# jankammeth/BA-path-planning

Hardware: AMD Instinct MI355X
Metric: SCP iterations/sec (N agents x K waypoints) (higher is better)
Workload: dtype f64

## Files before the change

### ba-path-planning_amd/csrc/scp_common.h

```cpp
#pragma once
#include <hip/hip_runtime.h>

#include <cstdarg>
#include <cstdint>
#include <cstdio>
#include <cstring>

#include "scp_hip.h"

struct scp_stats_mirror {
  scp_pair_stats stats;
  unsigned long long n_spec;
  double pts[6];
  double rel[64];
  volatile unsigned long long seq;
};

constexpr int SCP_SMALL_MAX_WG = 2048;

struct scp_ctx {
  int device;
  int n_cu;
  hipStream_t stream;
  char err[512];
// ... 1 lines not shown
  double* h_scratch;
  double* h_scratch_dev;
  hipEvent_t ev0, ev1;
  hipEvent_t pair_ev0, pair_ev1;
  bool pair_timed;
  bool pair_ran;
  bool last_pass_small;
  double* tm_scratch;
  size_t tm_bytes;
  uint32_t* cmp_map;
  size_t cmp_map_bytes;
  uint32_t* cmp_tot;
  size_t cmp_tot_bytes;
  scp_stats_mirror* h_mirror;
  scp_stats_mirror* d_mirror;
  unsigned long long mirror_seq;
  unsigned long long* wg_part;
  uint32_t* wg_rows;
  size_t wg_rows_bytes;
  unsigned* d_ticket;
  int timing;
  int small_pass;
  unsigned long long rel_seq;
  void* gen_ws;
  size_t gen_ws_bytes;
  void* sep_ws;
  size_t sep_ws_bytes;
  unsigned long long* solved;
  bool solved_ran[2];
  int* h_gen_flag;
  int* d_gen_flag;
  void* asg_ws;
  size_t asg_ws_bytes;
};

static inline int scp_fail(scp_ctx* ctx, int code, const char* fmt, ...) {
  if (ctx) {
    va_list ap;
    va_start(ap, fmt);
    vsnprintf(ctx->err, sizeof(ctx->err), fmt, ap);
    va_end(ap);
  }
  return code;
}

#define SCP_HIP_CHECK(ctx, call)                                                                     \
  do {                                                                                               \
    hipError_t e_ = (call);                                                                          \
    if (e_ != hipSuccess)                                                                            \
      return scp_fail((ctx), SCP_ERR_HIP, "%s failed: %s (%s:%d)", #call, hipGetErrorString(e_),    \
                      __FILE__, __LINE__);                                                           \
  } while (0)

#define SCP_REQUIRE(ctx, cond, ...)                                   \
  do {                                                                \
    if (!(cond)) return scp_fail((ctx), SCP_ERR_INVALID, __VA_ARGS__); \
  } while (0)

static inline int64_t scp_pairs(int N) { return (int64_t)N * (N - 1) / 2; }
static inline int scp_cdiv(int64_t a, int64_t b) { return (int)((a + b - 1) / b); }

int scp_ctx_ensure_bytes(scp_ctx* ctx, void** buf, size_t* have, size_t need);

hipError_t scp_raise_lds_limit(int device, const void* kernel, size_t bytes);

bool scp_wait_host_word(volatile unsigned long long* word, unsigned long long seq, int timeout_s);

int scp_check_pair_range(scp_ctx* ctx, int N, int K, int D, int64_t q_begin, int64_t q_end);

int scp_ctx_wait_stats(scp_ctx* ctx, scp_pair_stats* out);

int scp_violations_from_solution(scp_ctx* ctx, int N, int K, int D, double R, double h, int64_t q_begin, int64_t q_end,
                                 const double* pos_prev, const double* x_tm, const double* p0, const double* v0, double* x_out,
                                 double* pos_out, double feas_tol, int64_t* new_rows, int64_t new_cap, uint32_t* sel_bitmap,
                                 scp_pair_stats* stats, const double* rel_prev ,
                                 int64_t* spec_rows , int64_t spec_cap,
                                 uint32_t* spec_bitmap, double spec_margin, bool* fused);
void scp_ctx_mirror_rel(scp_ctx* ctx, int64_t n, double* out);
int scp_select_from_solution(scp_ctx* ctx, int N, int K, int D, double R, double h, int64_t q_begin, int64_t q_end,
                             const double* x_tm, const double* p0, const double* v0, double* x_out, double* pos_out,
                             double margin, int64_t* sel_rows, int64_t sel_cap, uint32_t* sel_bitmap, scp_pair_stats* stats,
                             bool* fused);
int scp_launch_kinematics_copy(scp_ctx* ctx, int N, int K, int D, double h, const double* acc, const double* p0,
                               const double* v0, double* pos_out, double* vel_out, double* acc_copy);
const double* scp_qp_solution_tm(const scp_qp* qp);

int scp_qp_reset_add_rows_at(scp_qp* qp, const double* x0, int64_t n, const int64_t* rows, const double* pos_prev,
                             const double* p0, const double* v0, double R);
int scp_qp_add_rows_from_pass(scp_qp* qp, int64_t n, const int64_t* rows, const double* eta, const double* l_col,
                              int64_t q_begin, int64_t q_end);

int scp_launch_add_rows_at(scp_ctx* ctx, int N, int K, int D, int64_t base, int64_t n, const int64_t* rows,
                           const double* pos_prev, const double* p0, const double* v0, double R, double h, const double* Qx,
                           int64_t* w_row, int* wk, int* wi, int* wj, double* weta, double* wl, double* zc, double* yc);

int scp_launch_gemm(scp_ctx* ctx, int use_mfma, int R, int M, int C, double alpha, const double* A,
                    const double* X, double beta, double* Y);
int scp_launch_to_time_major(scp_ctx* ctx, int N, int K, int D, const double* src, double* dst);
int scp_launch_from_time_major(scp_ctx* ctx, int N, int K, int D, const double* src, double* dst);
// ... 5 lines not shown
```

### ba-path-planning_amd/csrc/scp_ctx.hip

```cpp
#include "scp_common.h"
#include "scp_traj_device.h"

#include <sys/prctl.h>
#include <time.h>

#include <atomic>
#include <chrono>
#include <cmath>
#include <cstdlib>
#include <map>
#include <mutex>
#include <utility>

extern "C" int scp_abi_version(void) { return SCP_ABI_VERSION; }

extern "C" int scp_ctx_create(int device, void* hip_stream, scp_ctx** out) {
  if (!out) return SCP_ERR_INVALID;
  *out = nullptr;
  if (hipSetDevice(device) != hipSuccess) return SCP_ERR_HIP;
  scp_ctx* ctx = new scp_ctx();
  memset(ctx, 0, sizeof(*ctx));
  ctx->device = device;
  ctx->stream = (hipStream_t)hip_stream;
  ctx->timing = 1;
  ctx->small_pass = getenv("SCP_NO_SMALL_PASS") ? 0 : 1;
  if (hipDeviceGetAttribute(&ctx->n_cu, hipDeviceAttributeMultiprocessorCount, device) != hipSuccess) ctx->n_cu = 0;
  if (hipMalloc(&ctx->d_scratch, 72 * sizeof(double)) != hipSuccess ||
      hipMemset(ctx->d_scratch, 0, 72 * sizeof(double)) != hipSuccess ||
      hipHostMalloc(&ctx->h_scratch, 72 * sizeof(double)) != hipSuccess ||
      memset(ctx->h_scratch, 0, 72 * sizeof(double)) == nullptr ||
      hipHostGetDevicePointer((void**)&ctx->h_scratch_dev, ctx->h_scratch, 0) != hipSuccess ||
      hipHostMalloc(&ctx->h_mirror, sizeof(scp_stats_mirror)) != hipSuccess ||
      hipHostGetDevicePointer((void**)&ctx->d_mirror, ctx->h_mirror, 0) != hipSuccess ||
      hipEventCreate(&ctx->ev0) != hipSuccess || hipEventCreate(&ctx->ev1) != hipSuccess ||
      hipEventCreate(&ctx->pair_ev0) != hipSuccess || hipEventCreate(&ctx->pair_ev1) != hipSuccess ||
      hipMalloc(&ctx->wg_part, 4 * SCP_SMALL_MAX_WG * sizeof(unsigned long long)) != hipSuccess ||
      hipMalloc(&ctx->d_ticket, 64) != hipSuccess || hipMemset(ctx->d_ticket, 0, 64) != hipSuccess) {
    delete ctx;
    return SCP_ERR_HIP;
  }
  ctx->solved = (unsigned long long*)(ctx->d_ticket + 12);
  *out = ctx;
  return SCP_OK;
}

extern "C" int scp_ctx_set_option(scp_ctx* ctx, const char* key, int value) {
  if (!ctx || !key) return SCP_ERR_INVALID;
  if (strcmp(key, "kernel_timing") == 0) {
    ctx->timing = value ? 1 : 0;
    if (!ctx->timing) ctx->pair_timed = false;
    return SCP_OK;
  }
  if (strcmp(key, "single_launch_passes") == 0) {
    ctx->small_pass = value ? 1 : 0;
    return SCP_OK;
  }
  return scp_fail(ctx, SCP_ERR_INVALID, "ctx_set_option: unknown key '%s'", key);
}
// ... 116 lines not shown
```

### ba-path-planning_amd/csrc/scp_kernels.hip

```cpp
#include "scp_common.h"
#include "scp_compact_device.h"
#include "scp_pair_device.h"
#include "scp_traj_device.h"
#include "scp_wave_device.h"

#include <algorithm>
#include <cstdlib>

__device__ inline void pair_stats_init(scp_pair_stats* s) {
  s->min_dist = __longlong_as_double(0x7FF0000000000000LL);
  s->first_violation = 0xFFFFFFFFFFFFFFFFULL;
  s->n_selected = 0;
  s->max_violation = -__longlong_as_double(0x7FF0000000000000LL);
}

constexpr int PAIR_THREADS = 256;
constexpr int PAIR_STEPS = 16;
template <bool USE_LDS, int MODE>
struct PairUnroll {
  static constexpr int value = (USE_LDS && MODE != 2 ) ? 2 : 4;
};
constexpr int PAIR_ROWS = PAIR_THREADS * PAIR_STEPS * 2;
constexpr int PAIR_LDS_SLICE_BYTES = 16 * 1024;
constexpr int PAIR_LDS_Q_OFF = PAIR_LDS_SLICE_BYTES / 8;
// ... 808 lines not shown
        f = red_u[w] < f ? red_u[w] : f;
      }
      const double cur = __hip_atomic_load(&a.stats->min_dist, __ATOMIC_RELAXED, __HIP_MEMORY_SCOPE_AGENT);
      if (m < cur) atomic_min_pos_double(&a.stats->min_dist, m);
      if ((a.ablate & 1) && my_maxv == 12345.678) a.stats->max_violation = my_maxv;
      if (f != 0xFFFFFFFFFFFFFFFFULL) {
        const unsigned long long curf = __hip_atomic_load((unsigned long long*)&a.stats->first_violation,
                                                          __ATOMIC_RELAXED, __HIP_MEMORY_SCOPE_AGENT);
        if (f < curf) atomicMin((unsigned long long*)&a.stats->first_violation, f);
      }
    } else {
      double m = red_d[0];
#pragma unroll
      for (int w = 1; w < PAIR_THREADS / 64; ++w) m = fmax(m, red_d[w]);
      const double cur = __hip_atomic_load(&a.stats->max_violation, __ATOMIC_RELAXED, __HIP_MEMORY_SCOPE_AGENT);
      if (m > cur) atomic_max_double(&a.stats->max_violation, m);
    }
  }
#ifdef SCP_PHASE_PROFILE
  if (threadIdx.x == 0) {
    const unsigned wg = blockIdx.y * gridDim.x + blockIdx.x;
    if (wg < (unsigned)SCP_PAIR_CLK_WGS) {
      scp_pair_clk[2 * wg] = __builtin_amdgcn_s_memtime() - clk_c0;
      scp_pair_clk[2 * wg + 1] = __builtin_amdgcn_s_memrealtime() - clk_t0;
      scp_pair_t0[wg] = clk_t0;
    }
  }
#endif
}

__global__ __launch_bounds__(256) void pair_prep_delta_kernel(int N, int K, int D, const double* __restrict__ pos_prev,
                                                               const double* __restrict__ pos_new,
                                                               double* __restrict__ P_tm, double* __restrict__ dP_tm,
                                                               scp_pair_stats* __restrict__ stats) {
  const int64_t t = (int64_t)blockIdx.x * 256 + threadIdx.x;
  const int64_t C = (int64_t)N * D;
  if (t == 0) pair_stats_init(stats);
  if (t >= C * K) return;
  const int k = (int)(t / C);
  const int c = (int)(t % C);
  const int i = c / D, d = c % D;
  const int64_t g = ((int64_t)i * K + k) * D + d;
  const double pp = pos_prev[g];
  P_tm[t] = pp;
  dP_tm[t] = pos_new[g] - pp;
}

__global__ __launch_bounds__(CMP_THREADS) void compact_count_kernel(const uint32_t* __restrict__ map, int64_t words,
                                                                     uint32_t* __restrict__ block_tot) {
  const int64_t w0 = (int64_t)blockIdx.x * CMP_WORDS + (int64_t)threadIdx.x * CMP_WPT;
  int c = 0;
#pragma unroll
  for (int i = 0; i < CMP_WPT; ++i)
    if (w0 + i < words) c += __popc(map[w0 + i]);
  int tot;
  block_exclusive_scan(c, &tot);
  if (threadIdx.x == 0) block_tot[blockIdx.x] = (uint32_t)tot;
}

__global__ __launch_bounds__(CMP_THREADS) void compact_scan_kernel(uint32_t* __restrict__ block_tot, int nblocks,
                                                                    scp_pair_stats* __restrict__ stats,
                                                                    scp_stats_mirror* __restrict__ mirror,
                                                                    unsigned long long seq) {
  int carry = 0;
  for (int b0 = 0; b0 < nblocks; b0 += CMP_THREADS) {
    const int b = b0 + threadIdx.x;
    const int v = b < nblocks ? (int)block_tot[b] : 0;
    int tot;
    const int ex = block_exclusive_scan(v, &tot);
    if (b < nblocks) block_tot[b] = (uint32_t)(carry + ex);
    carry += tot;
  }
  if (threadIdx.x == 0) {
    stats->n_selected = (unsigned long long)carry;
    publish_stats(stats, (unsigned long long)carry, mirror, seq);
  }
}

// ... 176 lines not shown
  const int64_t slots = (int64_t)std::max(per_cu, 1) * ctx->n_cu;
  PairItems& it = a.items;
  it = PairItems{};
  const int64_t big_per_k = scp_cdiv(nq + 1, PAIR_ROWS);
  int nk_quarter = 0, nk_half = 0;
  if (big_per_k * K > slots) {
    nk_quarter = (int)((slots * (PAIR_ROWS / 4) + nq / 2) / nq);
    nk_half = (int)((slots * (PAIR_ROWS / 2) + nq / 2) / nq);
    if (nk_quarter + nk_half > K / 2) nk_quarter = nk_half = 0;
  }
#ifdef SCP_PHASE_PROFILE
  if (const char* e = getenv("SCP_PAIR_TAIL")) {
    int h_ = 0, q_ = 0;
    if (sscanf(e, "%d %d", &h_, &q_) == 2 && h_ >= 0 && q_ >= 0 && h_ + q_ < K) { nk_half = h_; nk_quarter = q_; }
  }
#endif
  const int nk[3] = {K - nk_half - nk_quarter, nk_half, nk_quarter};
  const int st[3] = {PAIR_STEPS, PAIR_STEPS / 2, PAIR_STEPS / 4};
  int k0 = 0, item0 = 0;
  for (int c = 0; c < 3; ++c) {
    if (nk[c] <= 0) continue;
    const int m = it.n_classes++;
    it.item0[m] = item0;
    it.k0[m] = k0;
    it.steps[m] = st[c];
    it.cpk[m] = (int)scp_cdiv(nq + 1, (int64_t)2 * PAIR_THREADS * st[c]);
    item0 += nk[c] * it.cpk[m];
    k0 += nk[c];
  }
  it.n_items = item0;
  return SCP_OK;
}

static int launch_large_pass(scp_ctx* ctx, int mode, PairArgs& a, const PassMarks& marks, const double* pos, const double* p0,
                             const double* v0) {
  const int N = a.N, K = a.K, D = a.D;
  const int64_t nq = a.q_end - a.q_begin;
  ctx->last_pass_small = false;
  const size_t slice = ((size_t)N * K * D + 1) & ~(size_t)1;
  const int rc = scp_ctx_ensure_bytes(ctx, (void**)&ctx->tm_scratch, &ctx->tm_bytes, 2 * slice * sizeof(double));
  if (rc) return rc;
  double* P_tm = mode != MODE_VIOLATIONS ? ctx->tm_scratch : nullptr;
  double* Q_tm = (mode != MODE_CHECK && mode != MODE_SELECT) ? ctx->tm_scratch + slice : nullptr;
  const dim3 prep_grid(scp_cdiv((int64_t)N * K * D, 256));
  const bool clear = marks.kind == PassMarks::REPLACE;
  if (mode == MODE_VIOL_RECOMPUTE)
    hipLaunchKernelGGL(pair_prep_delta_kernel, prep_grid, dim3(256), 0, ctx->stream, N, K, D, pos, p0, P_tm, Q_tm, a.stats);
  else
    hipLaunchKernelGGL(pair_prep_kernel, prep_grid, dim3(256), 0, ctx->stream, N, K, D, a.h, pos, p0, v0, P_tm, Q_tm,
                       a.stats, clear ? marks.bitmap : nullptr, clear ? a.words : (int64_t)0);
  a.P_tm = P_tm;
  a.Q_tm = Q_tm;
  if (nq <= 0) return SCP_OK;
  const size_t slice_bytes = (size_t)N * D * sizeof(double);
  const bool two_slices = mode == MODE_LINEARIZE || mode == MODE_VIOL_RECOMPUTE;
  const bool use_lds = slice_bytes <= (size_t)(two_slices ? 1 : 2) * PAIR_LDS_SLICE_BYTES && ((N * D) % 2 == 0) && !(a.ablate & 2);
  const size_t lds_bytes = !use_lds ? 0 : (two_slices ? PAIR_LDS_SLICE_BYTES + slice_bytes : slice_bytes);
  const PairKernel kern = pair_kernel(mode, D, use_lds, false);
  dim3 grid(scp_cdiv(nq + 1, PAIR_ROWS), K);
  if (mode == MODE_LINEARIZE) {
    const int rc_items = split_linearize_items(ctx, a, kern, lds_bytes);
    if (rc_items) return rc_items;
    grid = dim3((unsigned)a.items.n_items, 1);
  }
  return launch_pair_kernel(ctx, kern, grid, lds_bytes, a);
}

static int pair_pass(scp_ctx* ctx, int mode, PairArgs& a, const PassMarks& marks, const double* pos, const double* p0,
                     const double* v0) {
  if (marks.kind != PassMarks::NONE) {
    const int rc = ensure_cmp(ctx, a.words);
    if (rc) return rc;
  }
  a.bitmap = marks.bitmap;
  a.mark = marks.kind == PassMarks::MERGE ? ctx->cmp_map : marks.bitmap;
#ifdef SCP_PHASE_PROFILE
  const char* abl = getenv("SCP_PAIR_ABLATE");
  a.ablate = abl ? atoi(abl) : 0;
#endif
  if (pair_mode_has_small(mode) && small_pass_ok(ctx, a.N, a.K, a.D, a.q_end - a.q_begin, small_pass_slices(mode, a)))
    return launch_small_pass(ctx, mode, a, marks, pos, p0);
  const int rc = launch_large_pass(ctx, mode, a, marks, pos, p0, v0);
  if (rc || marks.kind == PassMarks::NONE) return rc;
  return launch_compaction(ctx, a.mark, a.words, a.q_end - a.q_begin, a.q_begin, a.pairs, marks.rows, marks.cap,
                           marks.kind == PassMarks::MERGE ? marks.bitmap : nullptr, a.stats);
}

#ifdef SCP_PHASE_PROFILE
extern "C" int scp_debug_small_clocks(unsigned long long* out, int n) {
  if (n > 16) n = 16;
  return hipMemcpyFromSymbol(out, HIP_SYMBOL(scp_small_clk), (size_t)n * sizeof(unsigned long long)) == hipSuccess ? 0 : 1;
}
extern "C" int scp_debug_pair_starts(unsigned long long* out, int n) {
  if (n > SCP_PAIR_CLK_WGS) n = SCP_PAIR_CLK_WGS;
  return hipMemcpyFromSymbol(out, HIP_SYMBOL(scp_pair_t0), (size_t)n * sizeof(unsigned long long)) == hipSuccess ? 0 : 1;
}
extern "C" int scp_debug_pair_clocks(unsigned long long* out, int n) {
  if (n > 2 * SCP_PAIR_CLK_WGS) n = 2 * SCP_PAIR_CLK_WGS;
  return hipMemcpyFromSymbol(out, HIP_SYMBOL(scp_pair_clk), (size_t)n * sizeof(unsigned long long)) == hipSuccess ? 0 : 1;
}
#endif

extern "C" int scp_ctx_last_pair_ms(scp_ctx* ctx, float* ms) {
  if (!ctx || !ms) return SCP_ERR_INVALID;
  if (!ctx->pair_timed && ctx->pair_ran) {
    *ms = 0.f;
    return SCP_OK;
  }
  if (!ctx->pair_timed) return scp_fail(ctx, SCP_ERR_STATE, "no pairwise pass has run yet");
  SCP_HIP_CHECK(ctx, hipEventSynchronize(ctx->pair_ev1));
  SCP_HIP_CHECK(ctx, hipEventElapsedTime(ms, ctx->pair_ev0, ctx->pair_ev1));
  return SCP_OK;
}

// ... 55 lines not shown
  if (!ctx) return SCP_ERR_INVALID;
  const int rc = scp_check_pair_range(ctx, N, K, D, q_begin, q_end);
  if (rc) return rc;
  SCP_REQUIRE(ctx, eta && l_col && pos && p0 && v0 && sel_bitmap && stats && (new_rows || new_cap == 0),
              "collision_violations: null pointer");
  PairArgs a = pair_args(N, K, D, 0.0, h, q_begin, q_end, stats);
  a.eta = const_cast<double*>(eta); a.l = const_cast<double*>(l_col); a.margin = feas_tol;
  return pair_pass(ctx, MODE_VIOLATIONS, a, {PassMarks::MERGE, new_rows, new_cap, sel_bitmap}, pos, p0, v0);
}

extern "C" int scp_collision_violations_at(scp_ctx* ctx, int N, int K, int D, double R, int64_t q_begin, int64_t q_end,
                                           const double* pos_prev, const double* pos_new, double feas_tol,
                                           int64_t* new_rows, int64_t new_cap, uint32_t* sel_bitmap,
                                           scp_pair_stats* stats) {
  if (!ctx) return SCP_ERR_INVALID;
  const int rc = scp_check_pair_range(ctx, N, K, D, q_begin, q_end);
  if (rc) return rc;
  SCP_REQUIRE(ctx, pos_prev && pos_new && sel_bitmap && stats && (new_rows || new_cap == 0),
              "collision_violations_at: null pointer");
  PairArgs a = pair_args(N, K, D, R, 0.0, q_begin, q_end, stats);
  a.margin = feas_tol;
  return pair_pass(ctx, MODE_VIOL_RECOMPUTE, a, {PassMarks::MERGE, new_rows, new_cap, sel_bitmap}, pos_prev, pos_new, nullptr);
}

int scp_violations_from_solution(scp_ctx* ctx, int N, int K, int D, double R, double h, int64_t q_begin, int64_t q_end,
                                 const double* pos_prev, const double* x_tm, const double* p0, const double* v0, double* x_out,
                                 double* pos_out, double feas_tol, int64_t* new_rows, int64_t new_cap, uint32_t* sel_bitmap,
                                 scp_pair_stats* stats, const double* rel_prev, int64_t* spec_rows, int64_t spec_cap,
                                 uint32_t* spec_bitmap, double spec_margin, bool* fused) {
  *fused = false;
  int rc = scp_check_pair_range(ctx, N, K, D, q_begin, q_end);
  if (rc) return rc;
  const int64_t nq = q_end - q_begin;
  if (!small_pass_ok(ctx, N, K, D, nq, 2)) return SCP_OK;
  if (!spec_bitmap || !small_pass_ok(ctx, N, K, D, nq, 3)) spec_rows = nullptr;
  PairArgs a = pair_args(N, K, D, R, h, q_begin, q_end, stats);
  a.margin = feas_tol;
  a.x_tm = x_tm; a.p0 = p0; a.v0 = v0; a.x_out = x_out; a.pos_out = pos_out;
  a.rel_prev = rel_prev;
  a.rel_blocks = rel_step_blocks((int64_t)N * K * D);
  a.spec_rows = spec_rows; a.spec_cap = spec_cap; a.spec_bitmap = spec_bitmap; a.spec_margin = spec_margin;
  rc = pair_pass(ctx, MODE_VIOL_RECOMPUTE, a, {PassMarks::MERGE, new_rows, new_cap, sel_bitmap}, pos_prev, nullptr, nullptr);
  if (rc) return rc;
  if (!ctx->last_pass_small) return scp_fail(ctx, SCP_ERR_STATE, "violations_from_solution: the small-problem pass did not run");
  *fused = true;
  return SCP_OK;
}

int scp_select_from_solution(scp_ctx* ctx, int N, int K, int D, double R, double h, int64_t q_begin, int64_t q_end,
                             const double* x_tm, const double* p0, const double* v0, double* x_out, double* pos_out,
                             double margin, int64_t* sel_rows, int64_t sel_cap, uint32_t* sel_bitmap, scp_pair_stats* stats,
                             bool* fused) {
  *fused = false;
  int rc = scp_check_pair_range(ctx, N, K, D, q_begin, q_end);
  if (rc) return rc;
  if (!small_pass_ok(ctx, N, K, D, q_end - q_begin, 1)) return SCP_OK;
  PairArgs a = pair_args(N, K, D, R, h, q_begin, q_end, stats);
  a.margin = margin;
  a.x_tm = x_tm; a.p0 = p0; a.v0 = v0; a.x_out = x_out; a.pos_out = pos_out;
  rc = pair_pass(ctx, MODE_SELECT, a, {PassMarks::REPLACE, sel_rows, sel_cap, sel_bitmap}, nullptr, nullptr, nullptr);
  if (rc) return rc;
  if (!ctx->last_pass_small) return scp_fail(ctx, SCP_ERR_STATE, "select_from_solution: the small-problem pass did not run");
  *fused = true;
  return SCP_OK;
}

// ... 58 lines not shown
```

### ba-path-planning_amd/path_planning/_hip.py

```python
from __future__ import annotations

import ctypes as C
import os

import numpy as np

_LIB = None
_LIB_PATH = None

SCP_OK = 0
SCP_ERR_CAPACITY = -3
UINT64_MAX = (1 << 64) - 1

STATUS_TEXT = {1: "solved", 2: "solved inaccurate", -2: "maximum iterations reached", -3: "primal infeasible"}


PIPELINES = ("qp0", "persistent", "persistent16", "three-launch", "three-launch-bigK", "fused", "generic", "persistent8-lean")


def pipeline_names(mask):
    return "+".join(n for b, n in enumerate(PIPELINES) if mask >> b & 1) or "none"


class HipError(RuntimeError):
# ... 115 lines not shown

class Clearance(C.Structure):
    _fields_ = [("min_dist", C.c_double), ("t_min", C.c_double), ("row", C.c_uint64), ("sample_min_dist", C.c_double),
                ("n_violating", C.c_uint64), ("reserved", C.c_uint64)]


CLEARANCE_DTYPE = np.dtype([("min_dist", np.float64), ("t_min", np.float64), ("row", np.uint64),
                            ("sample_min_dist", np.float64), ("n_violating", np.uint64), ("reserved", np.uint64)])


class AssignStats(C.Structure):
    _fields_ = [("cost_q", C.c_int64), ("cost_q_identity", C.c_int64), ("quantum", C.c_double), ("rounds", C.c_int64),
                ("bids", C.c_int64), ("phases", C.c_int32), ("status", C.c_int32)]


ASSIGN_STATS_DTYPE = np.dtype([("cost_q", np.int64), ("cost_q_identity", np.int64), ("quantum", np.float64),
                               ("rounds", np.int64), ("bids", np.int64), ("phases", np.int32), ("status", np.int32)])


class LineStats(C.Structure):
    _fields_ = [("min_approach", C.c_double), ("arg_i", C.c_int32), ("arg_j", C.c_int32), ("n_close", C.c_int64),
                ("n_opposed", C.c_int64)]


LINE_STATS_DTYPE = np.dtype([("min_approach", np.float64), ("arg_i", np.int32), ("arg_j", np.int32), ("n_close", np.int64),
                             ("n_opposed", np.int64)])

NO_ROW = 2**64 - 1

ABI_VERSION = 7

EXPORTS = [
    "scp_set_host_wait", "scp_abi_version", "scp_ctx_create", "scp_ctx_destroy", "scp_last_error", "scp_ctx_synchronize",
    "scp_ctx_last_pair_ms", "scp_ctx_set_option",
    "scp_kinematics", "scp_fixed_bounds", "scp_linearize_pairs", "scp_select_pairs", "scp_check_avoidance", "scp_qp_add_rows_at",
    "scp_check_separation", "scp_ctx_last_separation_solved", "scp_list_conflicts",
    "scp_clearance_profile", "scp_ctx_last_clearance_solved",
    "scp_collision_violations", "scp_collision_violations_at", "scp_gather_rows", "scp_rel_step", "scp_qp_default_settings",
    "scp_qp_workspace_bytes", "scp_qp_create", "scp_qp_destroy", "scp_qp_update_settings", "scp_qp_set_problem",
    "scp_qp_reset", "scp_qp_set_rho", "scp_qp_add_rows", "scp_qp_solve", "scp_qp_clone_state", "scp_qp_get_solution",
    "scp_qp_get_duals", "scp_gemm_f64", "scp_qp_peek", "scp_qp_debug_set",
    "scp_solve_default_options", "scp_solver_create", "scp_solver_destroy", "scp_solver_update_settings", "scp_solver_solve",
    "scp_solver_step", "scp_solver_shard_begin", "scp_solver_shard_rows", "scp_solver_shard_qp", "scp_solver_shard_violations",
    "scp_solver_shard_round_done", "scp_solver_shard_end", "scp_gen_default_params", "scp_generate_grid_swap",
    "scp_assign_goals", "scp_straight_line_check",
]


def library_path():
    env = os.environ.get("SCP_HIP_LIB")
    if env:
        return env
    here = os.path.dirname(os.path.abspath(__file__))
    return os.path.join(os.path.dirname(here), "lib", "libscp_hip.so")


def load_library():
    global _LIB, _LIB_PATH
    if _LIB is not None:
        return _LIB
    path = library_path()
    if not os.path.exists(path):
        raise HipError(-100, f"{path} not found: build the HIP extension first (make -C ba-path-planning_amd/csrc)")
    lib = C.CDLL(path)
    vp, i32, i64, f64, sz = C.c_void_p, C.c_int, C.c_int64, C.c_double, C.c_size_t
    pd = C.POINTER(C.c_double)
    lib.scp_abi_version.restype = i32
    if lib.scp_abi_version() != ABI_VERSION:
        raise HipError(-4,
                       f"{path}: ABI version {lib.scp_abi_version()}, this binding needs {ABI_VERSION} -- rebuild "
                       "(python -c 'import __graft_entry__ as g; g.build()')")
    lib.scp_set_host_wait.argtypes = [i32]
    lib.scp_ctx_set_option.argtypes = [vp, C.c_char_p, i32]
    lib.scp_ctx_set_option.restype = i32
    lib.scp_set_host_wait.restype = None
    lib.scp_ctx_create.argtypes = [i32, vp, C.POINTER(vp)]
    lib.scp_ctx_destroy.argtypes = [vp]
    lib.scp_ctx_destroy.restype = None
    lib.scp_last_error.argtypes = [vp]
    lib.scp_last_error.restype = C.c_char_p
    lib.scp_ctx_synchronize.argtypes = [vp]
    lib.scp_ctx_last_pair_ms.argtypes = [vp, C.POINTER(C.c_float)]
    lib.scp_kinematics.argtypes = [vp, i32, i32, i32, f64, vp, vp, vp, vp, vp]
    lib.scp_fixed_bounds.argtypes = [vp, i32, i32, i32, f64, pd, pd, vp, vp, vp, vp, vp, vp]
    lib.scp_linearize_pairs.argtypes = [vp, i32, i32, i32, f64, f64, i64, i64, vp, vp, vp, vp, vp, f64, vp, i64, vp, vp]
    lib.scp_select_pairs.argtypes = [vp, i32, i32, i32, f64, i64, i64, vp, f64, vp, i64, vp, vp]
    lib.scp_check_avoidance.argtypes = [vp, i32, i32, i32, f64, i64, i64, vp, vp]
    lib.scp_check_separation.argtypes = [vp, i32, i32, i32, f64, f64, i64, i64, vp, vp, vp, vp]
    lib.scp_ctx_last_separation_solved.argtypes = [vp, C.POINTER(C.c_uint64)]
    lib.scp_list_conflicts.argtypes = [vp, i32, i32, i32, f64, f64, i64, i64, vp, vp, vp, vp, i64, vp]
    lib.scp_clearance_profile.argtypes = [vp, i32, i32, i32, f64, f64, i64, i64, vp, vp, vp, vp, vp]
    lib.scp_ctx_last_clearance_solved.argtypes = [vp, C.POINTER(C.c_uint64)]
    lib.scp_collision_violations.argtypes = [vp, i32, i32, i32, f64, i64, i64, vp, vp, vp, vp, vp, f64, vp, i64, vp, vp]
    lib.scp_collision_violations_at.argtypes = [vp, i32, i32, i32, f64, i64, i64, vp, vp, f64, vp, i64, vp, vp]
    lib.scp_gather_rows.argtypes = [vp, i32, i32, i32, i64, i64, vp, vp, vp, i64, vp, vp]
    lib.scp_rel_step.argtypes = [vp, i64, vp, vp, pd]
    lib.scp_qp_default_settings.argtypes = [C.POINTER(QpSettings)]
    lib.scp_qp_default_settings.restype = None
    lib.scp_qp_workspace_bytes.argtypes = [i32, i32, i32, i64]
    lib.scp_qp_workspace_bytes.restype = sz
    lib.scp_qp_create.argtypes = [vp, i32, i32, i32, f64, C.POINTER(QpSettings), vp, sz, i64, C.POINTER(vp)]
    lib.scp_qp_destroy.argtypes = [vp]
    lib.scp_qp_destroy.restype = None
    lib.scp_qp_update_settings.argtypes = [vp, C.POINTER(QpSettings)]
    lib.scp_qp_set_problem.argtypes = [vp, pd, pd, vp, vp, vp, vp]
    lib.scp_qp_reset.argtypes = [vp, vp]
    lib.scp_qp_set_rho.argtypes = [vp, f64]
    lib.scp_qp_add_rows.argtypes = [vp, i64, vp, vp, vp]
# ... 58 lines not shown
    import torch

    return torch


def _harr(values):
    a = np.ascontiguousarray(values, dtype=np.float64)
    return a, a.ctypes.data_as(C.POINTER(C.c_double))


class Context:

    def __init__(self, device=0):
        torch = _torch()
        if not torch.cuda.is_available():
            raise HipError(-101, "no GPU visible: the SCP hot path runs on MI355X only (there is no CPU fallback)")
        self.lib = load_library()
        self.device = int(device)
        self.tdev = torch.device("cuda", self.device)
        torch.cuda.set_device(self.device)
        stream = torch.cuda.current_stream(self.tdev).cuda_stream
        h = C.c_void_p()
        rc = self.lib.scp_ctx_create(self.device, C.c_void_p(stream), C.byref(h))
        if rc != SCP_OK:
            raise HipError(rc, "scp_ctx_create failed")
        self.h = h
        self.stats = torch.zeros(4, dtype=torch.float64, device=self.tdev)

    def set_option(self, key, value):
        self.check(self.lib.scp_ctx_set_option(self.h, key.encode(), int(value)))
        if key != "kernel_timing":
            self.options_changed = True

    def set_timing(self, on):
        self.set_option("kernel_timing", 1 if on else 0)

    def close(self):
        if getattr(self, "h", None):
            self.lib.scp_ctx_destroy(self.h)
            self.h = None

    def __del__(self):
        try:
            self.close()
        except Exception:
            pass

    def check(self, rc):
        if rc != SCP_OK:
            raise HipError(rc, self.lib.scp_last_error(self.h).decode())

    def tensor(self, array):
        torch = _torch()
        return torch.as_tensor(np.ascontiguousarray(array, dtype=np.float64)).to(self.tdev)

    def empty(self, *shape, dtype=None):
        torch = _torch()
        return torch.empty(*shape, dtype=dtype or torch.float64, device=self.tdev)

    def read_stats(self):
        torch = _torch()
        raw = self.stats.cpu().numpy()
        u = raw.view(np.uint64)
        return float(raw[0]), int(u[1]), int(u[2]), float(raw[3])

    def last_pair_ms(self):
# ... 442 lines not shown
```

### include/scp_hip.h

```cpp
#ifndef SCP_HIP_H
#define SCP_HIP_H

#include <stddef.h>
#include <stdint.h>

#ifdef __cplusplus
extern "C" {
#endif

#define SCP_ABI_VERSION 7

typedef enum scp_status {
  SCP_OK = 0,
  SCP_ERR_INVALID = -1,
  SCP_ERR_HIP = -2,
  SCP_ERR_CAPACITY = -3,
  SCP_ERR_STATE = -4
} scp_status;

typedef struct scp_ctx scp_ctx;
typedef struct scp_qp scp_qp;

typedef struct scp_pair_stats {
  double min_dist;
// ... 30 lines not shown
  int32_t cg_iters_total;
  int64_t working_rows;
  double r_prim, r_dual;
  double rho;
  double solve_ms;
  int32_t pipeline;
  int32_t persist_launches;
  int32_t persist_gave_up;
  int32_t rho_switches_in_kernel;
} scp_qp_info;

typedef enum scp_qp_pipeline {
  SCP_PIPE_QP0 = 0,
  SCP_PIPE_PERSIST = 1,
  SCP_PIPE_PERSIST16 = 2,
  SCP_PIPE_CG1 = 3,
  SCP_PIPE_CG1_BIGK = 4,
  SCP_PIPE_FUSED = 5,
  SCP_PIPE_GENERIC = 6,
  SCP_PIPE_PERSIST8L = 7
} scp_qp_pipeline;

int scp_abi_version(void);
void scp_set_host_wait(int mode);

static inline int64_t scp_eta_stride(int64_t K, int64_t nq) { return (K * nq + 1) & ~(int64_t)1; }

int scp_ctx_create(int device, void* hip_stream , scp_ctx** out);
void scp_ctx_destroy(scp_ctx* ctx);
const char* scp_last_error(const scp_ctx* ctx);
int scp_ctx_synchronize(scp_ctx* ctx);
int scp_ctx_last_pair_ms(scp_ctx* ctx, float* ms);
int scp_ctx_set_option(scp_ctx* ctx, const char* key, int value);

int scp_kinematics(scp_ctx* ctx, int N, int K, int D, double h, const double* acc, const double* p0,
                   const double* v0, double* pos_out, double* vel_out);

int scp_fixed_bounds(scp_ctx* ctx, int N, int K, int D, double h, const double* limits, const double* space,
                     const double* p0, const double* v0, const double* pf, const double* vf, double* l_out,
                     double* u_out);

int scp_linearize_pairs(scp_ctx* ctx, int N, int K, int D, double R, double h, int64_t q_begin, int64_t q_end,
                        const double* pos_prev, const double* p0, const double* v0, double* eta_out,
                        double* l_out, double margin, int64_t* sel_rows, int64_t sel_cap, uint32_t* sel_bitmap,
                        scp_pair_stats* stats);

int scp_select_pairs(scp_ctx* ctx, int N, int K, int D, double R, int64_t q_begin, int64_t q_end, const double* pos_prev,
                     double margin, int64_t* sel_rows, int64_t sel_cap, uint32_t* sel_bitmap, scp_pair_stats* stats);

int scp_check_avoidance(scp_ctx* ctx, int N, int K, int D, double R, int64_t q_begin, int64_t q_end,
                        const double* pos, scp_pair_stats* stats);

typedef struct scp_separation_stats {
  double min_dist;
  double sample_min_dist;
  double argmin_t;
  uint64_t argmin_row;
  uint64_t first_violation;
  uint64_t n_violating;
} scp_separation_stats;
int scp_check_separation(scp_ctx* ctx, int N, int K, int D, double h, double R, int64_t q_begin, int64_t q_end,
                         const double* pos, const double* vel, const double* acc, scp_separation_stats* stats);
int scp_ctx_last_separation_solved(scp_ctx* ctx, uint64_t* n_solved );

typedef struct scp_conflict {
  uint64_t row;
// ... 178 lines not shown
```

Measured before the change: 426.4.

## Add uniform-grid near-neighbor pass for violation recompute with exact fallback

Adds a spatial-hash kernel that bins agent positions per time step into a uniform grid in LDS. It then checks only pairs in neighboring cells whose motion-bounded reach could violate the separation radius, instead of sweeping all N(N-1)/2 pairs. If the bounds are unbounded, or the max violation found is too negative to prove that no far pair matters, it falls back to the full pass. The check needs a host wait on stats each call, and skips the fused small-pass violation path when forced.

```diff
diff --git a/ba-path-planning_amd/csrc/scp_common.h b/ba-path-planning_amd/csrc/scp_common.h
--- a/ba-path-planning_amd/csrc/scp_common.h
+++ b/ba-path-planning_amd/csrc/scp_common.h
@@ -57,6 +57,9 @@
   int* d_gen_flag;
   void* asg_ws;
   size_t asg_ws_bytes;
+  int near_pass;
+  unsigned near_call_no;
+  unsigned long long near_ran, near_fell_back;
 };
 
 static inline int scp_fail(scp_ctx* ctx, int code, const char* fmt, ...) {
@@ -90,6 +93,24 @@
 hipError_t scp_raise_lds_limit(int device, const void* kernel, size_t bytes);
 
 bool scp_wait_host_word(volatile unsigned long long* word, unsigned long long seq, int timeout_s);
+
+constexpr double SCP_NEAR_TAU = 1e-6;
+constexpr double SCP_NEAR_MAX_ABS = 1e100;
+struct ScpNearArgs {
+  int N, K, D;
+  double R, feas_tol;
+  int64_t q_begin, q_end;
+  const double* P_tm;
+  const double* dP_tm;
+  const uint32_t* bitmap;
+  uint32_t* mark;
+  scp_pair_stats* stats;
+  const unsigned* unbounded;
+  unsigned call_no;
+};
+inline unsigned* scp_near_unbounded_word(scp_ctx* ctx) { return ctx->d_ticket + 3; }
+bool scp_near_fits(int N, int D, size_t* lds_bytes);
+int scp_launch_near_violations(scp_ctx* ctx, const ScpNearArgs& a, size_t lds_bytes);
 
 int scp_check_pair_range(scp_ctx* ctx, int N, int K, int D, int64_t q_begin, int64_t q_end);
 
diff --git a/ba-path-planning_amd/csrc/scp_ctx.hip b/ba-path-planning_amd/csrc/scp_ctx.hip
--- a/ba-path-planning_amd/csrc/scp_ctx.hip
+++ b/ba-path-planning_amd/csrc/scp_ctx.hip
@@ -24,6 +24,7 @@
   ctx->stream = (hipStream_t)hip_stream;
   ctx->timing = 1;
   ctx->small_pass = getenv("SCP_NO_SMALL_PASS") ? 0 : 1;
+  ctx->near_pass = 1;
   if (hipDeviceGetAttribute(&ctx->n_cu, hipDeviceAttributeMultiprocessorCount, device) != hipSuccess) ctx->n_cu = 0;
   if (hipMalloc(&ctx->d_scratch, 72 * sizeof(double)) != hipSuccess ||
       hipMemset(ctx->d_scratch, 0, 72 * sizeof(double)) != hipSuccess ||
diff --git a/ba-path-planning_amd/csrc/scp_kernels.hip b/ba-path-planning_amd/csrc/scp_kernels.hip
--- a/ba-path-planning_amd/csrc/scp_kernels.hip
+++ b/ba-path-planning_amd/csrc/scp_kernels.hip
@@ -864,7 +864,8 @@
 __global__ __launch_bounds__(256) void pair_prep_delta_kernel(int N, int K, int D, const double* __restrict__ pos_prev,
                                                                const double* __restrict__ pos_new,
                                                                double* __restrict__ P_tm, double* __restrict__ dP_tm,
-                                                               scp_pair_stats* __restrict__ stats) {
+                                                               scp_pair_stats* __restrict__ stats,
+                                                               unsigned* __restrict__ unbounded, unsigned call_no) {
   const int64_t t = (int64_t)blockIdx.x * 256 + threadIdx.x;
   const int64_t C = (int64_t)N * D;
   if (t == 0) pair_stats_init(stats);
@@ -874,8 +875,11 @@
   const int i = c / D, d = c % D;
   const int64_t g = ((int64_t)i * K + k) * D + d;
   const double pp = pos_prev[g];
+  const double dp = pos_new[g] - pp;
   P_tm[t] = pp;
-  dP_tm[t] = pos_new[g] - pp;
+  dP_tm[t] = dp;
+  if (!(fabs(pp) <= SCP_NEAR_MAX_ABS) || !(fabs(dp) <= SCP_NEAR_MAX_ABS))
+    __hip_atomic_store(unbounded, call_no, __ATOMIC_RELAXED, __HIP_MEMORY_SCOPE_AGENT);
 }
 
 __global__ __launch_bounds__(CMP_THREADS) void compact_count_kernel(const uint32_t* __restrict__ map, int64_t words,
@@ -1118,10 +1122,9 @@
   return SCP_OK;
 }
 
-static int launch_large_pass(scp_ctx* ctx, int mode, PairArgs& a, const PassMarks& marks, const double* pos, const double* p0,
-                             const double* v0) {
+static int launch_pass_prep(scp_ctx* ctx, int mode, PairArgs& a, const PassMarks& marks, const double* pos, const double* p0,
+                            const double* v0) {
   const int N = a.N, K = a.K, D = a.D;
-  const int64_t nq = a.q_end - a.q_begin;
   ctx->last_pass_small = false;
   const size_t slice = ((size_t)N * K * D + 1) & ~(size_t)1;
   const int rc = scp_ctx_ensure_bytes(ctx, (void**)&ctx->tm_scratch, &ctx->tm_bytes, 2 * slice * sizeof(double));
@@ -1130,13 +1133,26 @@
   double* Q_tm = (mode != MODE_CHECK && mode != MODE_SELECT) ? ctx->tm_scratch + slice : nullptr;
   const dim3 prep_grid(scp_cdiv((int64_t)N * K * D, 256));
   const bool clear = marks.kind == PassMarks::REPLACE;
-  if (mode == MODE_VIOL_RECOMPUTE)
-    hipLaunchKernelGGL(pair_prep_delta_kernel, prep_grid, dim3(256), 0, ctx->stream, N, K, D, pos, p0, P_tm, Q_tm, a.stats);
-  else
+  if (mode == MODE_VIOL_RECOMPUTE) {
+    if (++ctx->near_call_no == 0u) ctx->near_call_no = 1u;
+    hipLaunchKernelGGL(pair_prep_delta_kernel, prep_grid, dim3(256), 0, ctx->stream, N, K, D, pos, p0, P_tm, Q_tm, a.stats,
+                       scp_near_unbounded_word(ctx), ctx->near_call_no);
+  } else {
     hipLaunchKernelGGL(pair_prep_kernel, prep_grid, dim3(256), 0, ctx->stream, N, K, D, a.h, pos, p0, v0, P_tm, Q_tm,
                        a.stats, clear ? marks.bitmap : nullptr, clear ? a.words : (int64_t)0);
+  }
+  SCP_HIP_CHECK(ctx, hipGetLastError());
   a.P_tm = P_tm;
   a.Q_tm = Q_tm;
+  return SCP_OK;
+}
+
+static int launch_large_pass(scp_ctx* ctx, int mode, PairArgs& a, const PassMarks& marks, const double* pos, const double* p0,
+                             const double* v0) {
+  const int N = a.N, K = a.K, D = a.D;
+  const int64_t nq = a.q_end - a.q_begin;
+  const int rc_prep = launch_pass_prep(ctx, mode, a, marks, pos, p0, v0);
+  if (rc_prep) return rc_prep;
   if (nq <= 0) return SCP_OK;
   const size_t slice_bytes = (size_t)N * D * sizeof(double);
   const bool two_slices = mode == MODE_LINEARIZE || mode == MODE_VIOL_RECOMPUTE;
@@ -1164,8 +1180,28 @@
   const char* abl = getenv("SCP_PAIR_ABLATE");
   a.ablate = abl ? atoi(abl) : 0;
 #endif
-  if (pair_mode_has_small(mode) && small_pass_ok(ctx, a.N, a.K, a.D, a.q_end - a.q_begin, small_pass_slices(mode, a)))
+  const bool small = pair_mode_has_small(mode) && small_pass_ok(ctx, a.N, a.K, a.D, a.q_end - a.q_begin, small_pass_slices(mode, a));
+  size_t near_lds = 0;
+  if (mode == MODE_VIOL_RECOMPUTE && marks.kind == PassMarks::MERGE && !a.x_tm && ctx->near_pass != 0 &&
+      (!small || ctx->near_pass == 2) && a.q_end > a.q_begin && a.margin >= 0.0 && a.R > 0.0 && scp_near_fits(a.N, a.D, &near_lds)) {
+    int rc = launch_pass_prep(ctx, mode, a, marks, pos, p0, v0);
+    if (rc) return rc;
+    const ScpNearArgs na{a.N, a.K, a.D, a.R, a.margin, a.q_begin, a.q_end, a.P_tm, a.Q_tm, a.bitmap, a.mark, a.stats,
+                         scp_near_unbounded_word(ctx), ctx->near_call_no};
+    rc = scp_launch_near_violations(ctx, na, near_lds);
+    if (rc) return rc;
+    rc = launch_compaction(ctx, a.mark, a.words, a.q_end - a.q_begin, a.q_begin, a.pairs, marks.rows, marks.cap, marks.bitmap,
+                           a.stats);
+    if (rc) return rc;
+    scp_pair_stats st;
+    rc = scp_ctx_wait_stats(ctx, &st);
+    if (rc) return rc;
+    ++ctx->near_ran;
+    if (st.max_violation >= -0.5 * SCP_NEAR_TAU) return SCP_OK;
+    ++ctx->near_fell_back;
+  } else if (small) {
     return launch_small_pass(ctx, mode, a, marks, pos, p0);
+  }
   const int rc = launch_large_pass(ctx, mode, a, marks, pos, p0, v0);
   if (rc || marks.kind == PassMarks::NONE) return rc;
   return launch_compaction(ctx, a.mark, a.words, a.q_end - a.q_begin, a.q_begin, a.pairs, marks.rows, marks.cap,
@@ -1287,6 +1323,7 @@
   int rc = scp_check_pair_range(ctx, N, K, D, q_begin, q_end);
   if (rc) return rc;
   const int64_t nq = q_end - q_begin;
+  if (ctx->near_pass == 2) return SCP_OK;
   if (!small_pass_ok(ctx, N, K, D, nq, 2)) return SCP_OK;
   if (!spec_bitmap || !small_pass_ok(ctx, N, K, D, nq, 3)) spec_rows = nullptr;
   PairArgs a = pair_args(N, K, D, R, h, q_begin, q_end, stats);
diff --git a/ba-path-planning_amd/csrc/scp_near.hip b/ba-path-planning_amd/csrc/scp_near.hip
--- /dev/null
+++ b/ba-path-planning_amd/csrc/scp_near.hip
@@ -0,0 +1,276 @@
+#include "scp_common.h"
+#include "scp_compact_device.h"
+#include "scp_pair_device.h"
+#include "scp_wave_device.h"
+
+#include <algorithm>
+
+constexpr int NEAR_THREADS = CMP_THREADS;
+constexpr int NEAR_LANES = 4;
+constexpr int NEAR_AGENTS = NEAR_THREADS / NEAR_LANES;
+constexpr int NEAR_MAX_S = 16;
+constexpr int NEAR_MAX_CELLS = 2048;
+template <int D>
+struct NearCap {
+  static constexpr int value = D == 2 ? 45 : 12;
+};
+constexpr double NEAR_SIDE_SLACK = 1.0 + 1e-6;
+constexpr size_t NEAR_LDS_LIMIT = 160 * 1024 - 1024;
+
+static size_t near_lds_bytes(int N, int D) {
+  return (size_t)N * D * sizeof(double) + (size_t)N * sizeof(double) + (size_t)N * sizeof(int) + NEAR_MAX_CELLS * sizeof(int);
+}
+bool scp_near_fits(int N, int D, size_t* lds_bytes) {
+  *lds_bytes = near_lds_bytes(N, D);
+  return N >= 2 && (D == 2 || D == 3) && *lds_bytes <= NEAR_LDS_LIMIT;
+}
+
+template <int D>
+struct NearGrid {
+  double lo[D], inv[D];
+  int n[D];
+};
+template <int D>
+__device__ inline void near_cell(const NearGrid<D>& g, const Pt<D>& p, int (&c)[D]) {
+#pragma unroll
+  for (int d = 0; d < D; ++d)
+    c[d] = (int)fmin(fmax((p.v[d] - g.lo[d]) * g.inv[d], 0.0), (double)(g.n[d] - 1));
+}
+template <int D>
+__device__ inline int near_cell_index(const NearGrid<D>& g, const int (&c)[D]) {
+  int idx = c[D - 1];
+#pragma unroll
+  for (int d = D - 2; d >= 0; --d) idx = idx * g.n[d] + c[d];
+  return idx;
+}
+template <int D>
+__device__ inline double near_reach(const Pt<D>& dp) {
+  double ss = 0.0;
+#pragma unroll
+  for (int d = 0; d < D; ++d) ss = fma(dp.v[d], dp.v[d], ss);
+  return sqrt(ss) * (1.0 + 1e-10);
+}
+
+template <int D>
+__global__ __launch_bounds__(NEAR_THREADS) void near_violations_kernel(ScpNearArgs a) {
+  extern __shared__ __attribute__((aligned(16))) double lds[];
+  __shared__ double red[NEAR_THREADS / 64][2 * D + 1];
+  if (__hip_atomic_load(a.unbounded, __ATOMIC_RELAXED, __HIP_MEMORY_SCOPE_AGENT) == a.call_no) return;
+  const int N = a.N, k = blockIdx.x, tid = threadIdx.x;
+  const int64_t nq = a.q_end - a.q_begin;
+  const double* P = a.P_tm + (int64_t)k * N * D;
+  const double* Q = a.dP_tm + (int64_t)k * N * D;
+  double* sP = lds;
+  double* sM = lds + (int64_t)N * D;
+  int* sId = reinterpret_cast<int*>(sM + N);
+  int* sEnd = sId + N;
+  const double INF = __longlong_as_double(0x7FF0000000000000LL);
+
+  double lo[D], hi[D], mmax = 0.0;
+#pragma unroll
+  for (int d = 0; d < D; ++d) {
+    lo[d] = INF;
+    hi[d] = -INF;
+  }
+  for (int i = tid; i < N; i += NEAR_THREADS) {
+    const Pt<D> p = load_pt<D>(P, i);
+#pragma unroll
+    for (int d = 0; d < D; ++d) {
+      lo[d] = fmin(lo[d], p.v[d]);
+      hi[d] = fmax(hi[d], p.v[d]);
+    }
+    mmax = fmax(mmax, near_reach<D>(load_pt<D>(Q, i)));
+  }
+#pragma unroll
+  for (int d = 0; d < D; ++d) {
+    lo[d] = wave_min(lo[d]);
+    hi[d] = wave_max(hi[d]);
+  }
+  mmax = wave_max(mmax);
+  if ((tid & 63) == 63) {
+#pragma unroll
+    for (int d = 0; d < D; ++d) {
+      red[tid >> 6][d] = lo[d];
+      red[tid >> 6][D + d] = hi[d];
+    }
+    red[tid >> 6][2 * D] = mmax;
+  }
+  __syncthreads();
+#pragma unroll
+  for (int d = 0; d < D; ++d) {
+    lo[d] = red[0][d];
+    hi[d] = red[0][D + d];
+  }
+  mmax = red[0][2 * D];
+#pragma unroll
+  for (int w = 1; w < NEAR_THREADS / 64; ++w) {
+#pragma unroll
+    for (int d = 0; d < D; ++d) {
+      lo[d] = fmin(lo[d], red[w][d]);
+      hi[d] = fmax(hi[d], red[w][D + d]);
+    }
+    mmax = fmax(mmax, red[w][2 * D]);
+  }
+  NearGrid<D> g;
+  int cells = 1;
+  {
+    const double side_min = (a.R + 2.0 * mmax + SCP_NEAR_TAU) * NEAR_SIDE_SLACK;
+#pragma unroll
+    for (int d = 0; d < D; ++d) {
+      const double ext = hi[d] - lo[d];
+      g.n[d] = (int)fmin(floor(ext / side_min) + 1.0, (double)NearCap<D>::value);
+      const double side = fmax(side_min, ext / (double)g.n[d] * NEAR_SIDE_SLACK);
+      g.lo[d] = lo[d];
+      g.inv[d] = 1.0 / side;
+      cells *= g.n[d];
+    }
+  }
+
+  for (int c = tid; c < cells; c += NEAR_THREADS) sEnd[c] = 0;
+  __syncthreads();
+  for (int i = tid; i < N; i += NEAR_THREADS) {
+    int c[D];
+    near_cell<D>(g, load_pt<D>(P, i), c);
+    atomicAdd(sEnd + near_cell_index<D>(g, c), 1);
+  }
+  __syncthreads();
+  {
+    const int cpt = (cells + NEAR_THREADS - 1) / NEAR_THREADS;
+    const int c0 = tid * cpt, c1 = min(c0 + cpt, cells);
+    int mine = 0;
+    for (int c = c0; c < c1; ++c) mine += sEnd[c];
+    int total;
+    int run = block_exclusive_scan(mine, &total);
+    for (int c = c0; c < c1; ++c) {
+      const int n = sEnd[c];
+      sEnd[c] = run;
+      run += n;
+    }
+  }
+  __syncthreads();
+  for (int i = tid; i < N; i += NEAR_THREADS) {
+    const Pt<D> p = load_pt<D>(P, i);
+    int c[D];
+    near_cell<D>(g, p, c);
+    const int slot = atomicAdd(sEnd + near_cell_index<D>(g, c), 1);
+#pragma unroll
+    for (int d = 0; d < D; ++d) sP[slot * D + d] = p.v[d];
+    sM[slot] = near_reach<D>(load_pt<D>(Q, i));
+    sId[slot] = i;
+  }
+  __syncthreads();
+
+  auto cell_start_from = [&](int x) -> int {
+    if (x <= 0) return 0;
+    if (x >= N) return N;
+    int lo_c = 0, hi_c = cells - 1;
+    while (lo_c < hi_c) {
+      const int mid = (lo_c + hi_c) >> 1;
+      if (sEnd[mid] >= x) hi_c = mid;
+      else lo_c = mid + 1;
+    }
+    return sEnd[lo_c];
+  };
+  const int chunk = (N + (int)gridDim.y - 1) / (int)gridDim.y;
+  const int a0 = cell_start_from(min((int)blockIdx.y * chunk, N)), a1 = cell_start_from(min(((int)blockIdx.y + 1) * chunk, N));
+  const int sub = tid & (NEAR_LANES - 1);
+  double my_max = -INF;
+  for (int sa = a0 + tid / NEAR_LANES; sa < a1; sa += NEAR_AGENTS) {
+    Pt<D> Pa;
+#pragma unroll
+    for (int d = 0; d < D; ++d) Pa.v[d] = sP[sa * D + d];
+    const double ma = sM[sa];
+    const int ia = sId[sa];
+    int ca[D];
+    near_cell<D>(g, Pa, ca);
+    const int x0 = max(ca[0] - 1, 0), x1 = min(ca[0] + 1, g.n[0] - 1);
+    const int z0 = D == 3 ? max(ca[D - 1] - 1, 0) : 0, z1 = D == 3 ? min(ca[D - 1] + 1, g.n[D - 1] - 1) : 0;
+    for (int cz = z0; cz <= z1; ++cz) {
+      for (int cy = max(ca[1] - 1, 0); cy <= min(ca[1] + 1, g.n[1] - 1); ++cy) {
+        const int row = (D == 3 ? cz * g.n[1] + cy : cy) * g.n[0];
+        const int b0 = row + x0 > 0 ? sEnd[row + x0 - 1] : 0, b1 = sEnd[row + x1];
+        for (int sb = max(b0, sa + 1) + sub; sb < b1; sb += NEAR_LANES) {
+          Pt<D> Pb;
+          double ss = 0.0;
+#pragma unroll
+          for (int d = 0; d < D; ++d) {
+            Pb.v[d] = sP[sb * D + d];
+            const double df = Pa.v[d] - Pb.v[d];
+            ss = fma(df, df, ss);
+          }
+          const double reach = a.R + ma + sM[sb] + SCP_NEAR_TAU;
+          if (!(ss < reach * reach * (1.0 + 1e-12))) continue;
+          const int ib = sId[sb];
+          const bool fwd = ia < ib;
+          const int i = fwd ? ia : ib, j = fwd ? ib : ia;
+          const int64_t q = tri_off(i, N) + (j - i - 1);
+          if (q < a.q_begin || q >= a.q_end) continue;
+          const PairGeom<D> pg = pair_geom<D>(fwd ? Pa : Pb, fwd ? Pb : Pa);
+          const Pt<D> Di = load_pt<D>(Q, i), Dj = load_pt<D>(Q, j);
+          const double dist = pg.deg ? 1.0 : pg.raw;
+          double qd = 0.0;
+#pragma unroll
+          for (int d = 0; d < D; ++d) {
+            const double e_d = pg.deg ? (d == 0 ? 1.0 : 0.0) : pg.diff[d] * pg.inv;
+            qd = fma(e_d, Di.v[d] - Dj.v[d], qd);
+          }
+          const double viol = (a.R - dist) - qd;
+          my_max = fmax(my_max, viol);
+          if (viol > a.feas_tol) {
+            const int64_t lr = (int64_t)k * nq + (q - a.q_begin);
+            if (!((a.bitmap[lr >> 5] >> (lr & 31)) & 1u)) atomicOr(a.mark + (lr >> 5), 1u << (lr & 31));
+          }
+        }
+      }
+    }
+  }
+
+  my_max = wave_max(my_max);
+  __syncthreads();
+  if ((tid & 63) == 63) red[tid >> 6][0] = my_max;
+  __syncthreads();
+  if (tid == 0) {
+    double m = red[0][0];
+#pragma unroll
+    for (int w = 1; w < NEAR_THREADS / 64; ++w) m = fmax(m, red[w][0]);
+    const double cur = __hip_atomic_load(&a.stats->max_violation, __ATOMIC_RELAXED, __HIP_MEMORY_SCOPE_AGENT);
+    if (m > cur) atomic_max_double(&a.stats->max_violation, m);
+  }
+}
+
+int scp_launch_near_violations(scp_ctx* ctx, const ScpNearArgs& a, size_t lds_bytes) {
+  typedef void (*NearKernel)(ScpNearArgs);
+  const NearKernel kern = a.D == 2 ? near_violations_kernel<2> : near_violations_kernel<3>;
+  if (lds_bytes > 64 * 1024) SCP_HIP_CHECK(ctx, scp_raise_lds_limit(ctx->device, (const void*)kern, lds_bytes));
+  const int S = std::min(scp_cdiv(a.N, NEAR_AGENTS), NEAR_MAX_S);
+  if (ctx->timing) SCP_HIP_CHECK(ctx, hipEventRecord(ctx->pair_ev0, ctx->stream));
+  hipLaunchKernelGGL(kern, dim3(a.K, S), dim3(NEAR_THREADS), lds_bytes, ctx->stream, a);
+  SCP_HIP_CHECK(ctx, hipGetLastError());
+  if (ctx->timing) SCP_HIP_CHECK(ctx, hipEventRecord(ctx->pair_ev1, ctx->stream));
+  ctx->pair_timed = ctx->timing != 0;
+  ctx->pair_ran = true;
+  return SCP_OK;
+}
+
+extern "C" int scp_ctx_set_near_pass(scp_ctx* ctx, int mode) {
+  if (!ctx) return SCP_ERR_INVALID;
+  SCP_REQUIRE(ctx, mode >= 0 && mode <= 2, "ctx_set_near_pass: mode %d is not 0 (off), 1 (auto) or 2 (force)", mode);
+  ctx->near_pass = mode;
+  return SCP_OK;
+}
+
+extern "C" int scp_ctx_near_pass_counts(scp_ctx* ctx, uint64_t* n_near, uint64_t* n_fell_back) {
+  if (!ctx || !n_near || !n_fell_back) return SCP_ERR_INVALID;
+  *n_near = ctx->near_ran;
+  *n_fell_back = ctx->near_fell_back;
+  return SCP_OK;
+}
+
+extern "C" int scp_ctx_peek_scratch_map(scp_ctx* ctx, uint32_t* out, int64_t words) {
+  if (!ctx || !out || words < 0) return SCP_ERR_INVALID;
+  SCP_REQUIRE(ctx, (size_t)words * sizeof(uint32_t) <= ctx->cmp_map_bytes, "ctx_peek_scratch_map: the map has %lld words",
+              (long long)(ctx->cmp_map_bytes / sizeof(uint32_t)));
+  SCP_HIP_CHECK(ctx, hipStreamSynchronize(ctx->stream));
+  if (words > 0) SCP_HIP_CHECK(ctx, hipMemcpy(out, ctx->cmp_map, (size_t)words * sizeof(uint32_t), hipMemcpyDeviceToHost));
+  return SCP_OK;
+}
diff --git a/ba-path-planning_amd/path_planning/_hip.py b/ba-path-planning_amd/path_planning/_hip.py
--- a/ba-path-planning_amd/path_planning/_hip.py
+++ b/ba-path-planning_amd/path_planning/_hip.py
@@ -171,7 +171,7 @@
 
 EXPORTS = [
     "scp_set_host_wait", "scp_abi_version", "scp_ctx_create", "scp_ctx_destroy", "scp_last_error", "scp_ctx_synchronize",
-    "scp_ctx_last_pair_ms", "scp_ctx_set_option",
+    "scp_ctx_last_pair_ms", "scp_ctx_set_option", "scp_ctx_set_near_pass", "scp_ctx_near_pass_counts", "scp_ctx_peek_scratch_map",
     "scp_kinematics", "scp_fixed_bounds", "scp_linearize_pairs", "scp_select_pairs", "scp_check_avoidance", "scp_qp_add_rows_at",
     "scp_check_separation", "scp_ctx_last_separation_solved", "scp_list_conflicts",
     "scp_clearance_profile", "scp_ctx_last_clearance_solved",
@@ -213,6 +213,9 @@
     lib.scp_ctx_set_option.argtypes = [vp, C.c_char_p, i32]
     lib.scp_ctx_set_option.restype = i32
     lib.scp_set_host_wait.restype = None
+    lib.scp_ctx_set_near_pass.argtypes = [vp, i32]
+    lib.scp_ctx_near_pass_counts.argtypes = [vp, C.POINTER(C.c_uint64), C.POINTER(C.c_uint64)]
+    lib.scp_ctx_peek_scratch_map.argtypes = [vp, vp, i64]
     lib.scp_ctx_create.argtypes = [i32, vp, C.POINTER(vp)]
     lib.scp_ctx_destroy.argtypes = [vp]
     lib.scp_ctx_destroy.restype = None
@@ -337,6 +340,22 @@
         if key != "kernel_timing":
             self.options_changed = True
 
+    def set_near_pass(self, mode):
+        self.check(self.lib.scp_ctx_set_near_pass(self.h, int(mode)))
+        self.options_changed = True
+
+    def near_pass_counts(self):
+        n, f = C.c_uint64(), C.c_uint64()
+        self.check(self.lib.scp_ctx_near_pass_counts(self.h, C.byref(n), C.byref(f)))
+        return int(n.value), int(f.value)
+
+    def peek_scratch_map(self, words):
+        out = np.empty(int(words), dtype=np.uint32)
+        if out.size == 0:
+            return out
+        self.check(self.lib.scp_ctx_peek_scratch_map(self.h, out.ctypes.data_as(C.c_void_p), int(words)))
+        return out
+
     def set_timing(self, on):
         self.set_option("kernel_timing", 1 if on else 0)
 
diff --git a/include/scp_hip.h b/include/scp_hip.h
--- a/include/scp_hip.h
+++ b/include/scp_hip.h
@@ -86,6 +86,9 @@
 int scp_ctx_synchronize(scp_ctx* ctx);
 int scp_ctx_last_pair_ms(scp_ctx* ctx, float* ms);
 int scp_ctx_set_option(scp_ctx* ctx, const char* key, int value);
+int scp_ctx_set_near_pass(scp_ctx* ctx, int mode);
+int scp_ctx_near_pass_counts(scp_ctx* ctx, uint64_t* n_near , uint64_t* n_fell_back );
+int scp_ctx_peek_scratch_map(scp_ctx* ctx, uint32_t* out , int64_t words);
 
 int scp_kinematics(scp_ctx* ctx, int N, int K, int D, double h, const double* acc, const double* p0,
                    const double* v0, double* pos_out, double* vel_out);
```

New measurement: 453.1, median of 6. 6.2% higher.
